# MatchaChoco010/toy-cpu-pathtracing

Measured on AMD Instinct MI355X. Metric: Msamples/sec (whole node), scene3 MIS/Sobol 1920x1080, higher is better.
Workload: dtype f32; 1 GPU; scene3 1920x1080 mis+sobol, 1024-spp job, 1024 sample indices per step (BASELINE configs[1]); parallelism=single-gpu

## Files before the change

toy-cpu-pathtracing_amd/csrc/api.cpp:

```cpp
#include <hip/hip_runtime.h>

#include <algorithm>
#include <cmath>
#include <cstdio>
#include <cstring>
#include <string>
#include <vector>

#include "../../include/mi355pt.h"
#include "api_internal.hpp"

using namespace pt;

static thread_local std::string g_err;
bool pt::g_debug_unlocked = false;
int pt::fail(int code, const std::string& msg) { g_err = msg; return code; }

static const uint32_t CIE_CMF_BITS[470 * 4] = {
#include "cie_cmf.inc"
};
void pt::cie_cmf4(float out[470 * 4]) { std::memcpy(out, CIE_CMF_BITS, sizeof(CIE_CMF_BITS)); }

namespace {

// ... 64 lines not shown
}

static void free_parts(std::vector<MultiPart>& parts) {
    for (size_t i = 0; i < parts.size(); ++i) {
        MultiPart& m = parts[i];
        (void)hipSetDevice(m.device);
        if (m.stream) (void)hipStreamDestroy(m.stream);
        if (m.done) (void)hipEventDestroy(m.done);
        (void)hipFree(m.d_film); (void)hipFree(m.d_pack); (void)hipFree(m.d_stage); (void)hipFree(m.d_out);
        if (i > 0) delete m.scene;
    }
    parts.clear();
}
mi355pt_scene::~mi355pt_scene() {
    int cur = 0;
    const bool have = !parts.empty() && hipGetDevice(&cur) == hipSuccess;
    free_parts(parts);
    if (have) (void)hipSetDevice(cur);
    delete ctx;
}

static int launch_range(const mi355pt_scene* s, const mi355pt_camera* cam, const mi355pt_params* p, uint32_t s_begin, uint32_t s_end, float* d_accum,
                        hipStream_t stream, mi355pt_stats* stats, const PathOut& pout, int aov_kind, uint32_t illuminant_lut, const uint32_t* d_list,
                        uint32_t n_list) {
    const bool aov = aov_kind >= 0;
    if (!d_list && shard_tile_count(cam->width, cam->height, p->shard_index, p->shard_count) == 0) return MI355PT_OK;
    int rc;
    LaunchCtx* lc; int slot;
    if ((rc = get_launch_ctx(s, p->seed, &lc, &slot))) return rc;
    if (lc->device != s->impl.device) return fail(MI355PT_E_DEVICE, "launch context and scene live on different devices");
    const bool want_stats = stats && p->collect_stats;
    int& waves = aov ? lc->aov_waves[aov_kind] : lc->waves[want_stats ? 1 : 0][p->sampler & 1u][p->strategy < 3u ? p->strategy : 0u];
    if (!waves) waves = aov ? query_resident_waves_aov((uint32_t)aov_kind, s->impl.features)
                            : query_resident_waves(select_kernel(false, want_stats, s->impl.features, p->sampler, p->strategy));
    const DevCamera dc = make_camera(cam);
    LaunchPlan plan = d_list ? plan_launch_tiles(cam, p, s_begin, s_end, waves, n_list) : plan_launch(cam, p, s_begin, s_end, waves, aov);
    DevParams& dp = plan.params;
    if (d_list) set_tile_list(dp, d_list);
    unsigned* d_counter = lc->d_counters + slot;
    DevStats* d_stats = lc->d_stats + slot;
    HIP_TRY(hipMemsetAsync(d_counter, 0, sizeof(unsigned), stream));
    dp.stats_mode = p->collect_stats;
    if (want_stats || (aov && stats)) HIP_TRY(hipMemsetAsync(d_stats, 0, sizeof(DevStats), stream));
    hipEvent_t e0 = nullptr, e1 = nullptr;
    if (stats) { HIP_TRY(hipEventCreate(&e0)); HIP_TRY(hipEventCreate(&e1)); HIP_TRY(hipEventRecord(e0, stream)); }
    if ((rc = grow_device_buffer(&lc->d_partial, &lc->partial_bytes, plan.partial_floats * sizeof(float), stream))) return rc;
    const KernelKey key = select_kernel(d_list != nullptr, want_stats, s->impl.features, p->sampler, p->strategy);
    if ((rc = grow_device_buffer(&lc->d_defer, &lc->defer_bytes, aov ? (size_t)0 : query_defer_bytes_per_wave(key) * (size_t)plan.grid, stream))) return rc;
    if (aov) HIP_TRY(launch_aov((uint32_t)aov_kind, s->impl.dev, dc, dp, illuminant_lut, lc->d_hash, d_accum, d_counter, stats ? d_stats : nullptr,
                                s->impl.features, plan.grid, stream));
    else {
        DevScene dev = s->impl.dev;
        dev.cam_lists = use_camera_lists(key, dp.block_log2, camera_lists_enabled()) ? 1u : 0u;
        HIP_TRY(launch_pt(key, dev, dc, dp, plan.n_tiles,
                          lc->d_hash, d_accum, lc->d_partial, d_counter, d_list ? nullptr : d_stats, plan.grid, stream, pout, lc->d_defer));
    }
    if (stats) {
        HIP_TRY(hipEventRecord(e1, stream));
        HIP_TRY(hipEventSynchronize(e1));
        float ms = 0.0f;
        HIP_TRY(hipEventElapsedTime(&ms, e0, e1));
        std::memset(stats, 0, sizeof(*stats));
        stats->kernel_ms = ms; stats->launches = 1;
        if (want_stats || aov) {
            DevStats h;
            HIP_TRY(hipMemcpy(&h, d_stats, sizeof(h), hipMemcpyDeviceToHost));
            copy_stats(h, stats);
        }
        (void)hipEventDestroy(e0); (void)hipEventDestroy(e1);
    }
    return MI355PT_OK;
}

static int launch_ranges(const mi355pt_scene* s, const mi355pt_camera* cam, const mi355pt_params* p, uint32_t s_begin, uint32_t s_end, float* d_accum,
                         hipStream_t stream, mi355pt_stats* stats, const uint32_t* d_list, uint32_t n_list,
                         const PathOut& pout = PathOut{nullptr, nullptr, nullptr, 0u, 0u}, int aov_kind = -1, uint32_t illuminant_lut = 0) {
    return for_each_launch_range(p->sampler, stats != nullptr, s_begin, s_end, [&](uint32_t b, uint32_t e) {
        return launch_range(s, cam, p, b, e, d_accum, stream, stats, pout, aov_kind, illuminant_lut, d_list, n_list);
    });
}

int pt::render_accum_range(const mi355pt_scene* s, const mi355pt_camera* cam, const mi355pt_params* p, uint32_t s_begin, uint32_t s_end,
                           float* d_accum, void* hip_stream, mi355pt_stats* stats, const PathOut& pout, int aov_kind, uint32_t illuminant_lut) {
    const bool aov = aov_kind >= 0;
    int rc = check_args(s, cam, p, aov);
    if (rc) return rc;
    if (!d_accum || s_end > p->spp || s_begin >= s_end) return fail(MI355PT_E_INVALID, "bad sample range or null accumulator");
    if (aov) {
        if (aov_kind > MI355PT_AOV_SHADING_NORMAL) return fail(MI355PT_E_INVALID, "unknown AOV kind");
        if (p->collect_stats) return fail(MI355PT_E_INVALID, "the AOV renderers have no instrumented kernel: collect_stats must be 0");
        if (aov_kind == MI355PT_AOV_ALBEDO && illuminant_lut >= s->impl.luts.size())
            return fail(MI355PT_E_INVALID, "illuminant_lut is not a LUT470 id of this scene (presets::cie_illum_d6500())");
    }
    return launch_ranges(s, cam, p, s_begin, s_end, d_accum, (hipStream_t)hip_stream, stats, nullptr, 0u, pout, aov_kind, illuminant_lut);
}

static int check_tiles_args(const mi355pt_scene* s, const mi355pt_camera* cam, const mi355pt_params* p) {
    int rc = check_args(s, cam, p);
    if (rc) return rc;
    if (p->shard_count > 1u) return fail(MI355PT_E_INVALID, "tile lists name tiles of the whole frame: shard_count must be 0 or 1");
    if (p->collect_stats) return fail(MI355PT_E_INVALID, "there is no instrumented tile-list kernel: collect_stats must be 0");
    if (adaptive_tile_count(cam->width, cam->height) == 0u) return fail(MI355PT_E_INVALID, "the frame has 2^31 tiles or more");
    return MI355PT_OK;
}

extern "C" {
// ... 693 lines not shown
```

toy-cpu-pathtracing_amd/csrc/launch_plan.hpp:

```cpp
#pragma once
#include <algorithm>
#include <cmath>
#include <cstddef>
#include <cstdint>
#include <cstdlib>

#include "../../include/mi355pt.h"
#include "layout.hpp"

namespace pt {

struct V3 { float x, y, z; };
inline V3 cross3(V3 a, V3 b) { return {a.y * b.z - b.y * a.z, a.z * b.x - b.z * a.x, a.x * b.y - b.x * a.y}; }
inline V3 norm3(V3 a) { float r = 1.0f / std::sqrt((a.x * a.x) + (a.y * a.y) + (a.z * a.z)); return {a.x * r, a.y * r, a.z * r}; }

inline uint32_t log2_int(uint32_t v) { return v == 0 ? 0 : 31 - (uint32_t)__builtin_clz(v); }
inline uint32_t round_up_pow2(uint32_t v) { return v <= 1 ? 1 : 1u << (32 - __builtin_clz(v - 1)); }

inline uint32_t shard_tile_count(uint32_t width, uint32_t height, uint32_t shard_index, uint32_t shard_count) {
    const uint32_t total = ((width + 7) / 8) * ((height + 7) / 8);
    const uint32_t cnt = shard_count ? shard_count : 1u, idx = shard_count ? shard_index : 0u;
    return total > idx ? (total - idx + cnt - 1) / cnt : 0u;
}

// ... 100 lines not shown
    while (!aov && n_items * chunks < (uint32_t)waves * 8 && chunks * 2 <= n_samples &&
           (n_samples / (chunks * 2)) >= (n_items * chunks >= (uint32_t)waves ? 16u : 8u)) chunks *= 2;
#ifdef MI355PT_TUNING
    if (const char* e = getenv("MI355PT_CHUNKS")) { uint32_t c = (uint32_t)atoi(e); if (c >= 1 && c <= n_samples) chunks = c; }
#endif
    dp.chunks = chunks; dp.chunk_size = (n_samples + chunks - 1) / chunks;
    dp.n_work = n_items * chunks;
    dp.sample_prefix_digits = 0;
    if (dp.sampler == MI355PT_SAMPLER_SOBOL && block_log2 == 0 && (dp.log2_spp & 1u) == 0u && n_samples % chunks == 0) {
        const uint32_t cs = dp.chunk_size;
        uint32_t m = 0;
        while ((1u << (2u * (m + 1u))) <= cs) ++m;
        if ((1u << (2u * m)) == cs && s_begin % cs == 0 && m >= 3 && m <= dp.log2_spp / 2u &&
            2u * dp.n_base4_digits <= 2u * m + 27u) dp.sample_prefix_digits = dp.log2_spp / 2u - m;
    }
    const int grid = (int)std::min<uint32_t>(dp.n_work, (uint32_t)waves);
    return LaunchPlan{dp, n_tiles, grid, dp.chunks > 1 ? (size_t)n_tiles * dp.chunks * 64u * 3u : (size_t)0};
}
inline LaunchPlan plan_launch(const mi355pt_camera* cam, const mi355pt_params* p, uint32_t s_begin, uint32_t s_end, int waves, bool aov) {
    return plan_launch_over(cam, p, s_begin, s_end, waves, aov, shard_tile_count(cam->width, cam->height, p->shard_index, p->shard_count));
}
inline LaunchPlan plan_launch_tiles(const mi355pt_camera* cam, const mi355pt_params* p, uint32_t s_begin, uint32_t s_end, int waves, uint32_t n_list) {
    return plan_launch_over(cam, p, s_begin, s_end, waves, false, n_list);
}

enum : uint32_t { MODE_GENERIC = 0, MODE_MIS_SOBOL = 1, MODE_NEE_SOBOL = 2, MODE_PT = 3, MODE_COUNT = 4 };
#define PT_FOR_EACH_SET(P, C)                                                                                                          \
    P(0u) P(FEAT_TEX) P(FEAT_DIEL) P(FEAT_METAL) P(FEAT_DIEL | FEAT_ROUGH) P(FEAT_DELTA | FEAT_MLIGHT) P(FEAT_STD & ~FEAT_CC)           \
    C(FEAT_CC) C(FEAT_CC | FEAT_TEX) C(FEAT_STD) C(FEAT_ALL)
#define PT_NO_SET(F)
#define PT_FOR_EACH_PLAIN_SET(X) PT_FOR_EACH_SET(X, PT_NO_SET)
#define PT_FOR_EACH_CC_SET(X) PT_FOR_EACH_SET(PT_NO_SET, X)
#define PT_SET_ENTRY(F) (F),
inline constexpr uint32_t FEATURE_SETS[] = {PT_FOR_EACH_SET(PT_SET_ENTRY, PT_SET_ENTRY)};
inline constexpr uint32_t PLAIN_SETS[] = {PT_FOR_EACH_PLAIN_SET(PT_SET_ENTRY)};
inline constexpr uint32_t CC_SETS[] = {PT_FOR_EACH_CC_SET(PT_SET_ENTRY)};
#undef PT_SET_ENTRY
inline uint32_t pick_features(uint32_t feat) {
    for (uint32_t s : FEATURE_SETS) if ((feat & ~s) == 0u) return s;
    return FEAT_ALL;
}
struct KernelKey { bool tiles, stats; uint32_t mode, set; };
inline KernelKey select_kernel(bool tiles, bool stats, uint32_t feat, uint32_t sampler, uint32_t strategy) {
    if (stats) return KernelKey{tiles, true, MODE_GENERIC, (feat & (FEAT_CC | FEAT_EMTEX)) == 0u ? FEAT_STD & ~FEAT_CC : FEAT_ALL};
    const uint32_t mode = sampler == MI355PT_SAMPLER_SOBOL && strategy == MI355PT_STRATEGY_MIS ? MODE_MIS_SOBOL
                        : sampler == MI355PT_SAMPLER_SOBOL && strategy == MI355PT_STRATEGY_NEE ? MODE_NEE_SOBOL
                        : strategy == MI355PT_STRATEGY_PT ? MODE_PT : MODE_GENERIC;
    return KernelKey{tiles, false, mode, pick_features(feat)};
}

inline bool use_camera_lists(const KernelKey& key, uint32_t block_log2, bool enabled) { return enabled && !key.stats && block_log2 <= 3u; }
inline bool camera_lists_enabled() { const char* e = getenv("MI355PT_NO_CAMERA_LISTS"); return !(e && e[0] != '\0' && !(e[0] == '0' && e[1] == '\0')); }

}
```

toy-cpu-pathtracing_amd/csrc/layout.hpp:

```cpp
#pragma once
#include <stddef.h>
#include <stdint.h>

#if defined(__HIPCC__)
#define PT_HD __host__ __device__
#else
#define PT_HD
#endif

namespace pt {

#ifndef PT_STACK_DEPTH
#define PT_STACK_DEPTH 24
#endif
constexpr int STACK_DEPTH = PT_STACK_DEPTH;
constexpr int MAX_LEAF_TRIS = 4;
constexpr int MAX_BUILD_DEPTH = 22;
constexpr int HASH_TABLE_DIMS = 136;

struct alignas(16) DevNode {
    float bx[4];
    float by[4];
    float bz[4];
    int32_t child[2];
// ... 107 lines not shown
    uint32_t material;
    float area_sum;
    uint32_t kind;
    float intensity;
    float angle_inner, angle_outer;
    float pos[3];
    float pad0;
    float axis[3];
    float pad1;
};
static_assert(sizeof(DevLight) == 64, "light record");

struct DevEnv {
    const float* texels;
    const float* marginal;
    const float* conditional;
    uint32_t w, h;
    float total_weight, intensity;
    float l2r[9], r2l[9];
    uint32_t illuminant_lut;
    uint32_t light_index;
    uint32_t pad[2];
};

struct DevScene {
    const DevNode* nodes;
    const DevNode4* nodes4;
    const DevNode4Q* nodes4q;
    float grid_org[3], grid_cell[3];
    const DevTri* tris;
    const DevTriShade* shade;
    const DevTriLocal* tris_local;
    const DevTri* tris_render;
    float tri_shift[3]; uint32_t tris_are_local;
    float shared_mw[3]; uint32_t pad_mw;
    const DevInstance* instances;
    const DevMaterial* materials;
    const DevLight* lights;
    const DevLightTri* light_tris;
    const float* light_uvs;
    const float* luts;
    const float* cmf;
    const float* rgb2spec;
    const float* z_nodes;
    const uint32_t* texels;
    const DevTexture* textures;
    const float* cc_albedo;
    uint32_t n_nodes, n_tris, n_lights, n_materials;
    int32_t root;
    int32_t root4;
    uint32_t n_nodes4;
    uint32_t cam_lists;
    const DevEnv* envs;
    uint32_t n_envs, pad_env;
};

struct DevCamera {
    float s[3], u[3], f[3];
    float tan_half_fov, aspect;
    uint32_t width, height;
};

struct DevParams {
    uint32_t spp, seed, max_depth, strategy, sampler;
    float exposure;
    uint32_t log2_spp, n_base4_digits;
    uint32_t sample_begin, sample_end;
    uint32_t shard_index, shard_count;
    uint32_t tiles_x, tiles_y;
    uint32_t n_work;
    uint32_t chunks, chunk_size;
    uint32_t block_log2;
    uint32_t sample_prefix_digits;
    uint32_t stats_mode;
    uint32_t albedo_lut;
    float rr_gate;
    float xyz_to_rgb[9];
};
static_assert(offsetof(DevParams, shard_index) == 40 && offsetof(DevParams, shard_count) == 44, "the shard pair carries the tile-list pointer");
PT_HD inline void set_tile_list(DevParams& p, const uint32_t* list) {
    p.shard_index = (uint32_t)((uint64_t)(uintptr_t)list & 0xffffffffu); p.shard_count = (uint32_t)((uint64_t)(uintptr_t)list >> 32);
}
PT_HD inline const uint32_t* tile_list(const DevParams& p) { return (const uint32_t*)(uintptr_t)(((uint64_t)p.shard_count << 32) | p.shard_index); }

enum : uint32_t { FEAT_TEX = 1, FEAT_DIEL = 2, FEAT_CC = 4, FEAT_MLIGHT = 8, FEAT_ROUGH = 16, FEAT_METAL = 32, FEAT_DELTA = 64, FEAT_ENV = 128, FEAT_EMTEX = 256,
                  FEAT_STD = 255, FEAT_ALL = 511 };

struct DevStats {
    unsigned long long samples, closest_rays, shadow_rays, nodes_closest, tris_closest, nodes_shadow, tris_shadow;
    unsigned long long closest_hits, bounces, spectrum_evals, textured_lookups;
    unsigned long long phase_cycles[10];
    unsigned long long wave_steps[8];
    unsigned long long busy_hist[2][8];
    unsigned long long divergence[12];
};

}
```

toy-cpu-pathtracing_amd/csrc/pt_kernel_body.inc:

```
    __shared__ uint32_t s_stack[STACK_DEPTH * 64];
#ifndef PT_FILM_PIX
#define PT_FILM_PIX 64
#endif
    __shared__ float s_film[PT_FILM_PIX * 3];
    __shared__ uint32_t s_hi[SOBOL_HI_DIMS];
    __shared__ uint32_t s_p6[SOBOL_HI_DIMS];
    __shared__ unsigned s_work;
    constexpr bool PARK = (FEAT & FEAT_CC) != 0u && kernel_min_waves<FEAT>() <= 3;
    __shared__ float s_park[PARK ? 8 * 64 : 1];
    __shared__ uint8_t s_perm[96];
    __shared__ uint32_t s_ring[ANY_RING];
    __shared__ uint32_t s_occl[2];
    __shared__ uint32_t s_pair[64];
    const AnyLds any_lds{s_ring, s_occl, s_pair};
    __shared__ unsigned long long s_best[64];
    const ClosestLds closest_lds{s_ring, s_best, s_pair};
    __shared__ uint32_t s_infl[2];
    const PairLds pair_lds{s_ring, s_best, s_occl, s_pair, s_infl};
    constexpr bool CAMLIST = !STATS && tail_queue<FEAT, MODE>();
    __shared__ uint32_t s_cand[CAMLIST ? CAM_LIST_CAP : 1u];
    DevParams prm = prm_in;
    if constexpr (MODE == MODE_MIS_SOBOL) { prm.strategy = 2u; prm.sampler = 1u; }
    if constexpr (MODE == MODE_NEE_SOBOL) { prm.strategy = 1u; prm.sampler = 1u; }
    if constexpr (MODE == MODE_PT) prm.strategy = 0u;
    const uint32_t lane = threadIdx.x;
    auto park = [&](Path& Q, bool mine = true) {
        if constexpr (PARK) {
            if (mine) {
#pragma unroll
                for (int i = 0; i < 4; ++i) s_park[i * 64 + lane] = Q.pf[i];
                s_park[4 * 64 + lane] = Q.p_pdf; s_park[5 * 64 + lane] = Q.prev_pos.x; s_park[6 * 64 + lane] = Q.prev_pos.y; s_park[7 * 64 + lane] = Q.prev_pos.z;
            }
#pragma unroll
            for (int i = 0; i < 4; ++i) Q.pf[i] = 0.0f;
            Q.p_pdf = 0.0f; Q.prev_pos = mk3(0.0f, 0.0f, 0.0f);
        }
    };
    auto unpark = [&](Path& Q) {
        if constexpr (PARK) {
#pragma unroll
            for (int i = 0; i < 4; ++i) Q.pf[i] = s_park[i * 64 + lane];
            Q.p_pdf = s_park[4 * 64 + lane]; Q.prev_pos = mk3(s_park[5 * 64 + lane], s_park[6 * 64 + lane], s_park[7 * 64 + lane]);
        }
    };
    uint32_t* stack = s_stack + lane;
    for (uint32_t k = lane; k < 96u; k += 64u) s_perm[k] = (uint8_t)((perm_packed(k >> 2) >> (2u * (k & 3u))) & 3u);
    if constexpr ((FEAT & (FEAT_TEX | FEAT_EMTEX | FEAT_ENV)) != 0u) s_znodes[lane] = sc.z_nodes[lane];
    __syncthreads();
    SamplerCtx sctx{prm.sampler, prm.seed, prm.log2_spp, prm.n_base4_digits, cam.width, dim_hash_tab, nullptr, 0u, 0u, nullptr, s_perm};
    StatCounters st{};
    unsigned long long tp[10] = {0, 0, 0, 0, 0, 0, 0, 0, 0, 0};
    unsigned long long dvc[8] = {0, 0, 0, 0, 0, 0, 0, 0};
    unsigned long long t_loop0 = 0;
// ... 3 lines not shown
        if (lane == 0) s_work = atomicAdd(work_counter, 1u);
        __syncthreads();
        const uint32_t work = s_work;
        __syncthreads();
        if (work >= prm.n_work) break;
        const LaneJob job = PT_LANE_JOB(work, lane, cam, prm);
        const LaneJob job0 = PT_LANE_JOB(work, 0u, cam, prm);
        const uint32_t blk_log2 = prm.block_log2, blk_mask = (1u << blk_log2) - 1u;
        const uint32_t s_prefix = prm.sample_prefix_digits;
        const uint32_t hi_first_w = sobol_hi_first(prm.log2_spp, blk_log2) - s_prefix, hi_shift_w = 2u * hi_first_w - (prm.log2_spp & 1u);
        if (prm.sampler == 1u && hi_first_w < prm.n_base4_digits && hi_first_w >= 3u &&
            2u * prm.n_base4_digits - (prm.log2_spp & 1u) <= hi_shift_w + 27u) {
            sctx.hi_first = sobol_hi_first(prm.log2_spp, blk_log2) - s_prefix;
            sctx.hi_shift = 2u * sctx.hi_first - (prm.log2_spp & 1u);
            const uint32_t tile_m = (encode_morton2_u32(job0.px, job0.py) << prm.log2_spp) | (s_prefix ? job0.s_cur : 0u);
            for (uint32_t dmn = lane; dmn < (uint32_t)SOBOL_HI_DIMS; dmn += 64) {
                uint32_t e = (uint32_t)(sobol_tile_hi_digits(tile_m, dmn, prm.log2_spp, prm.n_base4_digits, sctx.hi_first) >> sctx.hi_shift);
                const uint64_t prefix = (uint64_t)tile_m >> sctx.hi_shift;
                e |= sobol_perm_index(prefix, dmn) << 27;
                uint32_t e6 = 0;
                for (uint32_t v7 = 0; v7 < 4u; ++v7) e6 |= sobol_perm_index((prefix << 2) | v7, dmn) << (5u * v7);
                s_hi[dmn] = e; s_p6[dmn] = e6;
            }
            sctx.hi_lds = s_hi; sctx.p6_lds = s_p6;
        }
        uint32_t cam_n = CAM_LIST_NONE;
        if constexpr (CAMLIST) {
            if (sc.cam_lists != 0u) {
                const uint32_t x0 = PT_CAM_UNIFORM(job0.px), y0 = PT_CAM_UNIFORM(job0.py);
                const CamWalk cw = cam_walk(sc.nodes4, sc.root4, sc.tris, sc.tri_shift, cam_pyramid(cam, x0, y0, x0 + blk_mask, y0 + blk_mask), s_cand, CAM_LIST_CAP, s_ring);
                cam_n = PT_CAM_UNIFORM(cw.overflow ? CAM_LIST_NONE : cw.count);
            }
        }
        if (lane < PT_FILM_PIX) { s_film[3 * lane] = 0.0f; s_film[3 * lane + 1] = 0.0f; s_film[3 * lane + 2] = 0.0f; }
        __syncthreads();
        const uint32_t n_s = job0.s_end > job0.s_cur ? job0.s_end - job0.s_cur : 0u;
        const uint32_t pool_size = n_s << (2u * blk_log2);
        uint32_t pool_next = 0u;
        uint32_t my_pix = lane;
        Path P{};
        park(P);
        bool active = false;
        constexpr bool MERGED = merged_traversal<FEAT, MODE>();
        ShadowReq sh{};
        bool dying = false, susp = false;
        CarryState carry{0ull};
        constexpr bool TAILQ = !STATS && tail_queue<FEAT, MODE>();
        constexpr uint32_t DEFER = TAILQ ? 0u : defer_classes<FEAT, MODE>();
        float4* const q_base = (DEFER != 0u || TAILQ) ? defer_buf + (size_t)blockIdx.x * (queue_bytes_per_wave(STATS, FEAT, MODE) / 16u) : nullptr;
        uint32_t q_head = 0u, q_tail = 0u;
        uint32_t q_count = 0u, q2_count = 0u;
        constexpr uint32_t TQ_CLASSES = (TAILQ && (FEAT & FEAT_CC) != 0u) ? ((1u << MT_CLEARCOAT) | (1u << (MT_CLEARCOAT | 8u))) : 0u;
        constexpr uint32_t QR = (TQ_CLASSES != 0u) ? QUEUE_RING : PT_TAILQ_RING1;
        while (true) {
            unsigned long long ts0 = 0, ts1 = 0, ts2 = 0, ts3 = 0, ts4 = 0, tsa = 0, tsb = 0;
            uint32_t bsdf_classes = 0u;
            if (STATS) ts0 = __builtin_amdgcn_s_memtime();
            bool popped = false;
            uint32_t pop_e = 0u;
            const unsigned long long m_needy = __ballot(!active);
            if (m_needy != 0ull && pool_next < pool_size) {
                const uint32_t idx = pool_next + rank_below(m_needy);
                if (!active && idx < pool_size) {
                    const uint32_t pix = idx & ((1u << (2u * blk_log2)) - 1u);
                    const uint32_t px = job0.px + (pix & blk_mask), py = job0.py + (pix >> blk_log2);
                    const uint32_t smp_i = job0.s_cur + (idx >> (2u * blk_log2));
                    const bool valid = px < cam.width && py < cam.height;
                    if (valid) { active = true; my_pix = pix; regen_path<STATS>(P, sctx, cam, px, py, smp_i, st); }
                }
                pool_next = min(pool_next + (uint32_t)__popcll(m_needy), pool_size);
            }
            if (!__any(active)) {
                if (pool_next >= pool_size && q_tail == q_head && (q_count | q2_count) == 0u) break;
                if (!((DEFER != 0u || TAILQ) && pool_next >= pool_size)) continue;
            }
            if (STATS) { ts1 = __builtin_amdgcn_s_memtime(); if (lane == 0) st.w[4]++; if (active) st.w[5]++; }
            Hit hit{};
            bool got = false;
            const bool canonical = STATS && prm.stats_mode == 1u;
            if (canonical) { if (active) got = trace_closest<STATS>(sc, P.ro, P.rd, 3.402823466e+38f, stack, hit, st); }
            else if constexpr (MERGED) {
                bool occluded = false;
                if (STATS && sh.on) st.w[6]++;
                bool cam_ray = false;
                if constexpr (CAMLIST) cam_ray = cam_n != CAM_LIST_NONE && active && !dying && P.from_camera && P.depth == 0u;
                if (!CAMLIST || __ballot((active && !dying && !popped && !cam_ray) || sh.on) != 0ull) {
                    PT_PRIO_TRAV_ENTER;
                    trace_pair_coop<STATS>(sc, P.ro, P.rd, active && !dying && !popped && !cam_ray, sh.o, sh.d, sh.t, sh.on, stack, lane, pair_lds, hit, got, occluded, st, &carry, susp, &susp);
                    PT_PRIO_TRAV_EXIT;
                }
                if constexpr (CAMLIST) {
                    if (__ballot(cam_ray) != 0ull) {
                        const RaySetup rs = setup_ray(P.rd);
                        const f3 o2 = tri_origin(sc, P.ro);
                        unsigned long long key = (0x7f7fffffull << 32) | 0xffffffffull;
                        for (uint32_t i = 0u; i < cam_n; ++i) {
                            const uint32_t tri = PT_CAM_UNIFORM(s_cand[i]);
                            const TriVerts tv = load_tri(sc.tris, tri);
                            float t, b0, b1, b2;
                            if (intersect_triangle<false>(o2, P.rd, rs.kx, rs.ky, rs.kz, rs.sx, rs.sy, rs.sz, 3.402823466e+38f, tv, t, b0, b1, b2)) {
                                const unsigned long long k = ((unsigned long long)__float_as_uint(t) << 32) | (unsigned long long)tri;
                                key = k < key ? k : key;
                            }
                        }
                        if (cam_ray) {
                            got = (uint32_t)key != 0xffffffffu;
                            if (got) winner_hit(sc, P.ro, P.rd, rs, (uint32_t)key, hit);
                        }
                    }
                }
                if (sh.on && !occluded) {
#pragma unroll
                    for (int i = 0; i < 4; ++i) P.L[i] = P.L[i] + sh.c[i];
                }
                sh = ShadowReq{};
            }
            else { PT_PRIO_TRAV_ENTER; got = trace_closest_coop<STATS>(sc, P.ro, P.rd, active, stack, lane, closest_lds, hit, st); PT_PRIO_TRAV_EXIT; }
            if (STATS) {
                const uint32_t mclass = (active && got) ? sc.materials[__float_as_uint(((const float4*)(sc.shade + hit.tri))[4].z)].type : 8u;
                uint32_t classes = 0u, largest = 0u, lanes = 0u;
                for (uint32_t c = 0u; c < 8u; ++c) {
                    const uint32_t n = (uint32_t)__popcll(__ballot(mclass == c));
                    classes += n ? 1u : 0u; largest = max(largest, n); lanes += n;
                }
                if (lane == 0 && lanes) { st.dv[0]++; st.dv[1] += classes; st.dv[2] += lanes; st.dv[3] += largest; }
                bsdf_classes = classes - (__ballot(mclass == MT_EMISSIVE) != 0ull ? 1u : 0u);
                ts2 = __builtin_amdgcn_s_memtime();
            }
            auto tq_store = [&](uint32_t e, const Path& Q, const Hit& h, uint32_t pix) {
                float4* r = q_base + (size_t)(e >> 8) * (TQ_F4 * QUEUE_RING) + (e & (QR - 1u));
                const uint32_t fl = (Q.wl.term ? 1u : 0u) | ((Q.depth & 1023u) << 1) | ((pix & 63u) << 11) | (Q.smp.dimension << 17);
                r[0u * QR] = make_float4(__uint_as_float(Q.smp.morton), __uint_as_float(fl), Q.wl.lam0, __uint_as_float(h.tri));
                r[1u * QR] = make_float4(Q.T[0], Q.T[1], Q.T[2], Q.T[3]);
                r[2u * QR] = make_float4(Q.L[0], Q.L[1], Q.L[2], Q.L[3]);
                r[3u * QR] = make_float4(Q.rd.x, Q.rd.y, Q.rd.z, h.b0);
                r[4u * QR] = make_float4(h.b1, h.b2, __uint_as_float(Q.smp.rkey_lo), __uint_as_float(Q.smp.rkey_hi));
            };
            auto tq_load = [&](uint32_t e, Path& Q, Hit& h, uint32_t& pix) {
                const float4* r = q_base + (size_t)(e >> 8) * (TQ_F4 * QUEUE_RING) + (e & (QR - 1u));
                const float4 a = r[0u * QR], b = r[1u * QR], c = r[2u * QR], d = r[3u * QR], e4 = r[4u * QR];
                const uint32_t fl = __float_as_uint(a.y);
                Q.smp.morton = __float_as_uint(a.x); Q.smp.dimension = fl >> 17; Q.smp.rkey_lo = __float_as_uint(e4.z); Q.smp.rkey_hi = __float_as_uint(e4.w);
                Q.wl.lam0 = a.z; Q.wl.term = (fl & 1u) != 0u; Q.depth = (fl >> 1) & 1023u; pix = (fl >> 11) & 63u;
                Q.from_camera = false; Q.prev_spec = false;
                Q.T[0] = b.x; Q.T[1] = b.y; Q.T[2] = b.z; Q.T[3] = b.w; Q.L[0] = c.x; Q.L[1] = c.y; Q.L[2] = c.z; Q.L[3] = c.w;
                Q.rd = mk3(d.x, d.y, d.z); Q.ro = mk3(0.0f, 0.0f, 0.0f);
                h.b0 = d.w; h.b1 = e4.x; h.b2 = e4.y; h.tri = __float_as_uint(a.w); h.mclass = 0u; h.t = 0.0f;
#pragma unroll
                for (int i = 0; i < 4; ++i) Q.pf[i] = 0.0f;
                Q.p_pdf = 0.0f; Q.prev_pos = mk3(0.0f, 0.0f, 0.0f);
            };
            auto dq_store = [&](uint32_t e, const Path& Q, const Hit& h, uint32_t pix) {
                float4* r = q_base + (size_t)e * DEFER_F4;
                const uint32_t fl = (Q.wl.term ? 1u : 0u) | (Q.from_camera ? 2u : 0u) | (Q.prev_spec ? 4u : 0u) | ((Q.depth & 1023u) << 3) | (pix << 16);
                r[0] = make_float4(__uint_as_float(Q.smp.morton), __uint_as_float(Q.smp.dimension), __uint_as_float(Q.smp.rkey_lo), __uint_as_float(Q.smp.rkey_hi));
                r[1] = make_float4(Q.wl.lam0, __uint_as_float(fl), Q.T[0], Q.T[1]);
                r[2] = make_float4(Q.T[2], Q.T[3], Q.L[0], Q.L[1]);
                r[3] = make_float4(Q.L[2], Q.L[3], Q.rd.x, Q.rd.y);
                r[4] = make_float4(Q.rd.z, Q.pf[0], Q.pf[1], Q.pf[2]);
                r[5] = make_float4(Q.pf[3], Q.p_pdf, Q.prev_pos.x, Q.prev_pos.y);
                r[6] = make_float4(Q.prev_pos.z, h.t, h.b0, h.b1);
                r[7] = make_float4(h.b2, __uint_as_float(h.tri), __uint_as_float(h.mclass), 0.0f);
            };
            auto dq_load = [&](uint32_t e, Path& Q, Hit& h, uint32_t& pix) {
                const float4* r = q_base + (size_t)e * DEFER_F4;
                const float4 a = r[0], b = r[1], c = r[2], d = r[3], e4 = r[4], f = r[5], g = r[6], h4 = r[7];
                const uint32_t fl = __float_as_uint(b.y);
                Q.smp.morton = __float_as_uint(a.x); Q.smp.dimension = __float_as_uint(a.y); Q.smp.rkey_lo = __float_as_uint(a.z); Q.smp.rkey_hi = __float_as_uint(a.w);
                Q.wl.lam0 = b.x; Q.wl.term = (fl & 1u) != 0u; Q.from_camera = (fl & 2u) != 0u; Q.prev_spec = (fl & 4u) != 0u; Q.depth = (fl >> 3) & 1023u; pix = fl >> 16;
                Q.T[0] = b.z; Q.T[1] = b.w; Q.T[2] = c.x; Q.T[3] = c.y; Q.L[0] = c.z; Q.L[1] = c.w; Q.L[2] = d.x; Q.L[3] = d.y;
                Q.rd = mk3(d.z, d.w, e4.x); Q.ro = mk3(0.0f, 0.0f, 0.0f);
                Q.pf[0] = e4.y; Q.pf[1] = e4.z; Q.pf[2] = e4.w; Q.pf[3] = f.x; Q.p_pdf = f.y; Q.prev_pos = mk3(f.z, f.w, g.x);
                h.t = g.y; h.b0 = g.z; h.b1 = g.w; h.b2 = h4.x; h.tri = __float_as_uint(h4.y); h.mclass = __float_as_uint(h4.z);
            };
            auto finish_path = [&]() {
                if (pout.L != nullptr) {
                    const uint32_t px = job0.px + (my_pix & blk_mask), py = job0.py + (my_pix >> blk_log2);
                    const uint32_t tile_k = (work / prm.chunks) >> (6u - 2u * blk_log2);
                    const uint32_t smp_i = P.smp.morton & ((1u << prm.log2_spp) - 1u);
                    sample_log(P, pout, ((size_t)tile_k * 64u + ((py & 7u) * 8u + (px & 7u))) * pout.n_s + (smp_i - pout.s_base));
                }
                float r, g, b;
                film_rgb(P, sc, prm, r, g, b);
                atomicAdd(&s_film[3 * my_pix], r); atomicAdd(&s_film[3 * my_pix + 1], g); atomicAdd(&s_film[3 * my_pix + 2], b);
            };
            if constexpr (TAILQ) {
                bool end_path = dying;
                const bool front = active && !dying && !susp;
                unpark(P);
                {
                    ShadeCtx C0;
                    C0.cont = false;
                    if (front) end_path = shade_vertex_head<STATS, FEAT, 1>(P, sc, prm, sctx, got, hit, sh, st, tsa, C0);
                }
                dying = false;
                const bool go_on = front && !end_path;
                const bool cls2 = TQ_CLASSES != 0u && ((TQ_CLASSES >> (hit.mclass & 31u)) & 1u) != 0u;
                const unsigned long long m_on1 = __ballot(go_on && !cls2), m_on2 = TQ_CLASSES != 0u ? __ballot(go_on && cls2) : 0ull;
                if ((m_on1 | m_on2) != 0ull) {
                    if (go_on) {
                        const uint32_t e = cls2 ? QUEUE_RING + tq_push_slot(q2_count, rank_below(m_on2)) : tq_push_slot(q_count, rank_below(m_on1));
                        tq_store(e, P, hit, my_pix);
                        active = false;
                    }
                    q_count += (uint32_t)__popcll(m_on1); q2_count += (uint32_t)__popcll(m_on2);
                    __builtin_amdgcn_fence(__ATOMIC_RELEASE, "workgroup");
                }
                if (active && end_path) { finish_path(); active = false; }
                park(P, false);
                if (STATS) ts3 = ts4 = __builtin_amdgcn_s_memtime();
                const bool draining = pool_next >= pool_size;
                if (tq_pass_due(q_count, q2_count, draining, TQ_CLASSES != 0u, (uint32_t)PT_TAILQ_MIN)) {
                    const unsigned long long m_free = __ballot(!active);
                    const uint32_t n_free = (uint32_t)__popcll(m_free), r = rank_below(m_free);
                    const TqTake tk = tq_pass_take(q_count, q2_count, n_free, draining, TQ_CLASSES != 0u, (uint32_t)PT_TAILQ_MIN);
                    const uint32_t n2 = tk.n2, n1 = tk.n1;
                    const bool take2 = !active && r < n2, take1 = !active && !take2 && r - n2 < n1;
                    const bool take = take1 || take2;
                    const uint32_t e = take2 ? QUEUE_RING + tq_pop_slot(q2_count, n2, r) : tq_pop_slot(q_count, n1, r - n2);
                    q2_count -= n2; q_count -= n1;
                    bool ep = false;
                    if constexpr ((FEAT & FEAT_CC) != 0u) {
                        ShadeCtx C;
                        shade_ctx_idle_cc(C);
                        if (take) {
                            __builtin_amdgcn_fence(__ATOMIC_ACQUIRE, "workgroup");
                            tq_load(e, P, hit, my_pix);
                            active = true;
                            shade_vertex_head<STATS, FEAT, 2>(P, sc, prm, sctx, true, hit, sh, st, tsa, C);
                        }
                        const bool want_mc = take && C.cont && C.need_cc;
                        const float fc_mc = coat_directional_albedo_coop(want_mc, C.cc_alpha_c, C.cc_r0c, C.wo_nm, C.mc_key, lane);
                        if (want_mc) C.cc_fc = fc_mc;
                        if (take && C.cont) ep = shade_vertex_tail<STATS, FEAT>(P, sc, prm, sctx, sh, st, tsb, C);
                    } else if (take) {
                        __builtin_amdgcn_fence(__ATOMIC_ACQUIRE, "workgroup");
                        tq_load(e, P, hit, my_pix);
                        active = true;
                        ShadeCtx C;
                        C.cont = false; C.need_cc = false; C.cc_fc = 0.0f;
                        shade_vertex_head<STATS, FEAT, 2>(P, sc, prm, sctx, true, hit, sh, st, tsa, C);
                        if (C.cont) ep = shade_vertex_tail<STATS, FEAT>(P, sc, prm, sctx, sh, st, tsb, C);
                    }
                    park(P, take);
                    if (sh.on && sh.c[0] == 0.0f && sh.c[1] == 0.0f && sh.c[2] == 0.0f && sh.c[3] == 0.0f) sh.on = false;
                    if (!active) sh.on = false;
                    if (take) { dying = sh.on && ep; if (dying) ep = false; }
                    if (take && ep) { finish_path(); active = false; }
                }
            } else
            for (int pass = 0;; ++pass) {
            const bool mine = pass == 0 || popped;
            bool end_path = pass == 0 && MERGED && dying;
            if (pass == 0) {
                if constexpr (!MERGED) sh = ShadowReq{};
                unpark(P);
            }
            if constexpr (DEFER != 0u) {
                if (popped) {
                    __builtin_amdgcn_fence(__ATOMIC_ACQUIRE, "workgroup");
                    dq_load(pop_e, P, hit, my_pix);
                    got = true;
                }
                const bool defer_now = pass == 0 && !(STATS && prm.stats_mode == 1u) && active && !dying && !susp && !popped && got && ((DEFER >> (hit.mclass & 31u)) & 1u) != 0u;
                const unsigned long long m_def = __ballot(defer_now);
                if (m_def != 0ull) {
                    if (defer_now) {
                        dq_store((q_tail + rank_below(m_def)) & (DEFER_RING - 1u), P, hit, my_pix);
                        active = false;
                    }
                    q_tail += (uint32_t)__popcll(m_def);
                    __builtin_amdgcn_fence(__ATOMIC_RELEASE, "workgroup");
                }
            }
            const bool shade_now = mine && active && !(MERGED && (dying || susp));
            if constexpr ((FEAT & FEAT_CC) != 0u) {
                ShadeCtx C;
                shade_ctx_idle_cc(C);
                if (shade_now) end_path = shade_vertex_head<STATS, FEAT>(P, sc, prm, sctx, got, hit, sh, st, tsa, C);
                const bool want_mc = shade_now && C.cont && C.need_cc;
                const float fc_mc = coat_directional_albedo_coop(want_mc, C.cc_alpha_c, C.cc_r0c, C.wo_nm, C.mc_key, lane);
                if (want_mc) C.cc_fc = fc_mc;
                if (shade_now && C.cont) end_path = shade_vertex_tail<STATS, FEAT>(P, sc, prm, sctx, sh, st, tsb, C);
            } else {
                if (shade_now) end_path = shade_vertex<STATS, FEAT>(P, sc, prm, sctx, got, hit, sh, st, tsa, tsb);
            }
            park(P, mine);
            if (STATS) {
                ts3 = __builtin_amdgcn_s_memtime();
                unsigned long long ma = __ballot(tsa != 0ull), mb = __ballot(tsb != 0ull);
// ... 76 lines not shown
```

toy-cpu-pathtracing_amd/csrc/scene_lower.cpp:

```cpp
#include "scene_lower.hpp"

#include <algorithm>
#include <cfloat>
#include <cmath>
#include <cstdio>
#include <cstring>

namespace pt {

namespace {

constexpr float PI_F = 3.14159265358979323846f;

struct V3 { float x, y, z; };
inline V3 operator-(V3 a, V3 b) { return {a.x - b.x, a.y - b.y, a.z - b.z}; }
inline V3 cross(V3 a, V3 b) { return {a.y * b.z - b.y * a.z, a.z * b.x - b.z * a.x, a.x * b.y - b.x * a.y}; }
inline float dot(V3 a, V3 b) { return (a.x * b.x) + (a.y * b.y) + (a.z * b.z); }
inline float length(V3 a) { return std::sqrt(dot(a, a)); }
inline V3 normalize(V3 a) { float r = 1.0f / length(a); return {a.x * r, a.y * r, a.z * r}; }
inline V3 vertex(const HostMesh& mesh, uint32_t v) { return V3{mesh.pos[3 * v], mesh.pos[3 * v + 1], mesh.pos[3 * v + 2]}; }
inline bool degenerate(V3 a, V3 b, V3 c) { const V3 cr = cross(b - a, c - a); return dot(cr, cr) == 0.0f; }

template <typename Rec>
inline void set_vertices(Rec& r, V3 a, V3 b, V3 c) {
// ... 547 lines not shown
    dev.n_envs = (uint32_t)ls->envs.size();
    dev.n_nodes = (uint32_t)ls->nodes.size(); dev.n_tris = (uint32_t)ls->tris_render.size();
    dev.n_lights = (uint32_t)ls->lights.size(); dev.n_materials = (uint32_t)ls->materials.size();
    dev.root = bvh.root;
    rep->n_degenerate = g.n_degenerate;
    rep->bvh_depth = bvh.max_depth;
    return MI355PT_OK;
}

int lower_tree4(LoweredScene* ls, LowerReport* rep, std::string* err) {
    std::vector<DevNode4> nodes4;
    if (!collapse_bvh4(ls->nodes, ls->dev.root, ls->tris_render.size(), &nodes4, &ls->dev.root4, &rep->stack_need, err, &rep->collapse_method)) return MI355PT_E_INVALID;
    ls->dev.n_nodes4 = (uint32_t)nodes4.size();
#if PT_NODE_FMA
    pad_nodes4(&nodes4);
#endif
#if PT_NODE_Q16
    if (!quantise_nodes4(nodes4, ls->dev.grid_org, ls->dev.grid_cell, &ls->nodes4, err)) return MI355PT_E_INVALID;
#else
    ls->nodes4 = std::move(nodes4);
#endif
    return MI355PT_OK;
}

std::string lowering_info(const LoweredScene& ls, const LowerReport& rep, bool gpu_builder, const double* ms) {
    char t_bvh[64] = "", t_collapse[32] = "", tail[160];
    if (ms) { std::snprintf(t_bvh, sizeof(t_bvh), " bvh_ms=%.2f bvh_device_ms=%.2f", ms[0], ms[1]); std::snprintf(t_collapse, sizeof(t_collapse), " collapse_ms=%.2f", ms[2]); }
    std::snprintf(tail, sizeof(tail), " stack_need=%d/%d degenerate=%zu tri_space=%s features=%u", rep.stack_need, STACK_DEPTH, rep.n_degenerate,
                  ls.dev.tris_are_local ? "local" : "render", ls.features);
    return "nodes4=" + std::to_string(ls.dev.n_nodes4) + " nodes=" + std::to_string(ls.nodes.size()) + " tris=" + std::to_string(ls.tris_render.size()) +
           " depth=" + std::to_string(rep.bvh_depth) + " builder=" + (gpu_builder ? "gpu" : "host") + t_bvh + " collapse=" + rep.collapse_method + t_collapse + tail;
}

void lowering_digests(const LoweredScene& ls, const LowerReport& rep, std::vector<std::string>* names, std::vector<uint64_t>* digests) {
    names->clear(); digests->clear();
    auto add = [&](const std::string& name, const void* p, size_t bytes) { names->push_back(name); digests->push_back(fnv1a64(p, bytes)); };
#define PT_DIGEST(v) add(#v, ls.v.data(), ls.v.size() * sizeof(ls.v[0]))
    PT_DIGEST(nodes); PT_DIGEST(nodes4); PT_DIGEST(tris_render); PT_DIGEST(shade); PT_DIGEST(instances); PT_DIGEST(tris_local); PT_DIGEST(cc_albedo);
    PT_DIGEST(materials); PT_DIGEST(lights); PT_DIGEST(light_tris); PT_DIGEST(light_uvs); PT_DIGEST(luts); PT_DIGEST(cmf); PT_DIGEST(rgb2spec);
    PT_DIGEST(z_nodes); PT_DIGEST(texels); PT_DIGEST(textures);
#undef PT_DIGEST
    for (size_t k = 0; k < ls.env_tables.size(); ++k) {
        const LoweredScene::EnvTables& t = ls.env_tables[k];
        const std::string e = "env" + std::to_string(k);
        add(e + ".texels", t.texels.data(), t.texels.size() * 4); add(e + ".marginal", t.marginal.data(), t.marginal.size() * 4);
        add(e + ".conditional", t.conditional.data(), t.conditional.size() * 4);
    }
    add("envs", ls.envs.data(), ls.envs.size() * sizeof(DevEnv));
    std::string b;
    auto put = [&](const void* p, size_t n) { b.append((const char*)p, n); };
    const DevScene& dev = ls.dev;
    put(dev.grid_org, 12); put(dev.grid_cell, 12); put(dev.tri_shift, 12); put(&dev.tris_are_local, 4); put(dev.shared_mw, 12); put(&dev.pad_mw, 4);
    put(&dev.n_nodes, 4); put(&dev.n_tris, 4); put(&dev.n_lights, 4); put(&dev.n_materials, 4); put(&dev.root, 4); put(&dev.root4, 4);
    put(&dev.n_nodes4, 4); put(&dev.cam_lists, 4); put(&dev.n_envs, 4); put(&dev.pad_env, 4);
    const uint32_t feat = ls.features; const uint64_t ndeg = rep.n_degenerate, nn4 = dev.n_nodes4; const int32_t depth = rep.bvh_depth, need = rep.stack_need;
    put(&feat, 4); put(&ndeg, 8); put(&depth, 4); put(&nn4, 8); put(&need, 4); put(rep.collapse_method, std::strlen(rep.collapse_method));
    add("scalars", b.data(), b.size());
}

}
```

toy-cpu-pathtracing_amd/csrc/tail_queue_plan.hpp:

```cpp
#pragma once
#include <cstdint>

namespace pt {

constexpr uint32_t tq_push_slot(uint32_t count, uint32_t rank) { return count + rank; }
constexpr uint32_t tq_pop_slot(uint32_t count, uint32_t n, uint32_t rank) { return count - n + rank; }

struct TqTake { uint32_t n1, n2; };

constexpr bool tq_pass_due(uint32_t c1, uint32_t c2, bool draining, bool two_queues, uint32_t pass_min) {
    return (two_queues && c2 >= pass_min) || c1 >= pass_min || (draining && (c1 | c2) != 0u);
}
constexpr TqTake tq_pass_take(uint32_t c1, uint32_t c2, uint32_t n_free, bool draining, bool two_queues, uint32_t pass_min) {
    const bool full2 = two_queues && c2 >= pass_min, full1 = c1 >= pass_min;
    const uint32_t n2 = (full2 || (draining && !full1)) ? (n_free < c2 ? n_free : c2) : 0u;
    const uint32_t n1 = (!full2 || draining) ? (n_free - n2 < c1 ? n_free - n2 : c1) : 0u;
    return TqTake{n1, n2};
}

}
```

Baseline: 2701 Msamples/s.

## Stage tail-queue pushes in LDS when a pass is due immediately

When the lanes pushed in this iteration would trigger a tail-queue pass straight away, their path records go into the LDS traversal-stack buffer instead of the global-memory ring. The following pop then reads those records back from LDS and the rest from global memory, which skips a global write and read round trip for records that are consumed at once. The LDS stack is reused as scratch, so its ordering against traversal has to stay correct. The staging is on by default for non-stats kernels with a single queue and can be turned off with an environment variable.

```diff
diff --git a/toy-cpu-pathtracing_amd/csrc/api.cpp b/toy-cpu-pathtracing_amd/csrc/api.cpp
--- a/toy-cpu-pathtracing_amd/csrc/api.cpp
+++ b/toy-cpu-pathtracing_amd/csrc/api.cpp
@@ -140,6 +140,7 @@
     else {
         DevScene dev = s->impl.dev;
         dev.cam_lists = use_camera_lists(key, dp.block_log2, camera_lists_enabled()) ? 1u : 0u;
+        dev.queue_stage = use_queue_staging(key, queue_staging_enabled()) ? 1u : 0u;
         HIP_TRY(launch_pt(key, dev, dc, dp, plan.n_tiles,
                           lc->d_hash, d_accum, lc->d_partial, d_counter, d_list ? nullptr : d_stats, plan.grid, stream, pout, lc->d_defer));
     }
diff --git a/toy-cpu-pathtracing_amd/csrc/launch_plan.hpp b/toy-cpu-pathtracing_amd/csrc/launch_plan.hpp
--- a/toy-cpu-pathtracing_amd/csrc/launch_plan.hpp
+++ b/toy-cpu-pathtracing_amd/csrc/launch_plan.hpp
@@ -176,4 +176,7 @@
 inline bool use_camera_lists(const KernelKey& key, uint32_t block_log2, bool enabled) { return enabled && !key.stats && block_log2 <= 3u; }
 inline bool camera_lists_enabled() { const char* e = getenv("MI355PT_NO_CAMERA_LISTS"); return !(e && e[0] != '\0' && !(e[0] == '0' && e[1] == '\0')); }
 
+inline bool use_queue_staging(const KernelKey& key, bool enabled) { return enabled && !key.stats; }
+inline bool queue_staging_enabled() { const char* e = getenv("MI355PT_NO_QUEUE_STAGING"); return !(e && e[0] != '\0' && !(e[0] == '0' && e[1] == '\0')); }
+
 }
diff --git a/toy-cpu-pathtracing_amd/csrc/layout.hpp b/toy-cpu-pathtracing_amd/csrc/layout.hpp
--- a/toy-cpu-pathtracing_amd/csrc/layout.hpp
+++ b/toy-cpu-pathtracing_amd/csrc/layout.hpp
@@ -183,7 +183,8 @@
     uint32_t n_nodes4;
     uint32_t cam_lists;
     const DevEnv* envs;
-    uint32_t n_envs, pad_env;
+    uint32_t n_envs;
+    uint32_t queue_stage;
 };
 
 struct DevCamera {
diff --git a/toy-cpu-pathtracing_amd/csrc/pt_kernel_body.inc b/toy-cpu-pathtracing_amd/csrc/pt_kernel_body.inc
--- a/toy-cpu-pathtracing_amd/csrc/pt_kernel_body.inc
+++ b/toy-cpu-pathtracing_amd/csrc/pt_kernel_body.inc
@@ -1,4 +1,4 @@
-    __shared__ uint32_t s_stack[STACK_DEPTH * 64];
+    __shared__ __attribute__((aligned(16))) uint32_t s_stack[STACK_DEPTH * 64];
 #ifndef PT_FILM_PIX
 #define PT_FILM_PIX 64
 #endif
@@ -108,6 +108,9 @@
         uint32_t q_count = 0u, q2_count = 0u;
         constexpr uint32_t TQ_CLASSES = (TAILQ && (FEAT & FEAT_CC) != 0u) ? ((1u << MT_CLEARCOAT) | (1u << (MT_CLEARCOAT | 8u))) : 0u;
         constexpr uint32_t QR = (TQ_CLASSES != 0u) ? QUEUE_RING : PT_TAILQ_RING1;
+        constexpr bool STAGE = TAILQ && TQ_CLASSES == 0u;
+        static_assert(STACK_DEPTH * 64 >= (int)(TQ_STAGE_SLOTS * TQ_F4 * 4u) && TQ_STAGE_SLOTS == 64u, "a pass's worth of staged tail-queue records fits the traversal stack's LDS");
+        float4* const s_stage = (float4*)s_stack;
         while (true) {
             unsigned long long ts0 = 0, ts1 = 0, ts2 = 0, ts3 = 0, ts4 = 0, tsa = 0, tsb = 0;
             uint32_t bsdf_classes = 0u;
@@ -183,18 +186,21 @@
                 bsdf_classes = classes - (__ballot(mclass == MT_EMISSIVE) != 0ull ? 1u : 0u);
                 ts2 = __builtin_amdgcn_s_memtime();
             }
+            auto tq_put = [&](float4* r, uint32_t stride, const Path& Q, const Hit& h, uint32_t pix) {
+                const uint32_t fl = (Q.wl.term ? 1u : 0u) | ((Q.depth & 1023u) << 1) | ((pix & 63u) << 11) | (Q.smp.dimension << 17);
+                r[0u * stride] = make_float4(__uint_as_float(Q.smp.morton), __uint_as_float(fl), Q.wl.lam0, __uint_as_float(h.tri));
+                r[1u * stride] = make_float4(Q.T[0], Q.T[1], Q.T[2], Q.T[3]);
+                r[2u * stride] = make_float4(Q.L[0], Q.L[1], Q.L[2], Q.L[3]);
+                r[3u * stride] = make_float4(Q.rd.x, Q.rd.y, Q.rd.z, h.b0);
+                r[4u * stride] = make_float4(h.b1, h.b2, __uint_as_float(Q.smp.rkey_lo), __uint_as_float(Q.smp.rkey_hi));
+            };
             auto tq_store = [&](uint32_t e, const Path& Q, const Hit& h, uint32_t pix) {
-                float4* r = q_base + (size_t)(e >> 8) * (TQ_F4 * QUEUE_RING) + (e & (QR - 1u));
-                const uint32_t fl = (Q.wl.term ? 1u : 0u) | ((Q.depth & 1023u) << 1) | ((pix & 63u) << 11) | (Q.smp.dimension << 17);
-                r[0u * QR] = make_float4(__uint_as_float(Q.smp.morton), __uint_as_float(fl), Q.wl.lam0, __uint_as_float(h.tri));
-                r[1u * QR] = make_float4(Q.T[0], Q.T[1], Q.T[2], Q.T[3]);
-                r[2u * QR] = make_float4(Q.L[0], Q.L[1], Q.L[2], Q.L[3]);
-                r[3u * QR] = make_float4(Q.rd.x, Q.rd.y, Q.rd.z, h.b0);
-                r[4u * QR] = make_float4(h.b1, h.b2, __uint_as_float(Q.smp.rkey_lo), __uint_as_float(Q.smp.rkey_hi));
-            };
-            auto tq_load = [&](uint32_t e, Path& Q, Hit& h, uint32_t& pix) {
-                const float4* r = q_base + (size_t)(e >> 8) * (TQ_F4 * QUEUE_RING) + (e & (QR - 1u));
-                const float4 a = r[0u * QR], b = r[1u * QR], c = r[2u * QR], d = r[3u * QR], e4 = r[4u * QR];
+                tq_put(q_base + (size_t)(e >> 8) * (TQ_F4 * QUEUE_RING) + (e & (QR - 1u)), QR, Q, h, pix);
+            };
+            struct TqRec { float4 a, b, c, d, e4; };
+            auto tq_get = [&](const float4* r, uint32_t stride) { return TqRec{r[0u * stride], r[1u * stride], r[2u * stride], r[3u * stride], r[4u * stride]}; };
+            auto tq_unpack = [&](const TqRec& rec, Path& Q, Hit& h, uint32_t& pix) {
+                const float4 a = rec.a, b = rec.b, c = rec.c, d = rec.d, e4 = rec.e4;
                 const uint32_t fl = __float_as_uint(a.y);
                 Q.smp.morton = __float_as_uint(a.x); Q.smp.dimension = fl >> 17; Q.smp.rkey_lo = __float_as_uint(e4.z); Q.smp.rkey_hi = __float_as_uint(e4.w);
                 Q.wl.lam0 = a.z; Q.wl.term = (fl & 1u) != 0u; Q.depth = (fl >> 1) & 1023u; pix = (fl >> 11) & 63u;
@@ -205,6 +211,9 @@
 #pragma unroll
                 for (int i = 0; i < 4; ++i) Q.pf[i] = 0.0f;
                 Q.p_pdf = 0.0f; Q.prev_pos = mk3(0.0f, 0.0f, 0.0f);
+            };
+            auto tq_load = [&](uint32_t e, Path& Q, Hit& h, uint32_t& pix) {
+                tq_unpack(tq_get(q_base + (size_t)(e >> 8) * (TQ_F4 * QUEUE_RING) + (e & (QR - 1u)), QR), Q, h, pix);
             };
             auto dq_store = [&](uint32_t e, const Path& Q, const Hit& h, uint32_t pix) {
                 float4* r = q_base + (size_t)e * DEFER_F4;
@@ -253,10 +262,19 @@
                 const bool go_on = front && !end_path;
                 const bool cls2 = TQ_CLASSES != 0u && ((TQ_CLASSES >> (hit.mclass & 31u)) & 1u) != 0u;
                 const unsigned long long m_on1 = __ballot(go_on && !cls2), m_on2 = TQ_CLASSES != 0u ? __ballot(go_on && cls2) : 0ull;
+                uint32_t n_on1 = 0u;
+                bool stage = false;
+                if constexpr (STAGE) {
+                    n_on1 = (uint32_t)__popcll(m_on1);
+                    stage = sc.queue_stage != 0u && tq_stage_pushes(q_count, n_on1, pool_next >= pool_size, (uint32_t)PT_TAILQ_MIN);
+                }
                 if ((m_on1 | m_on2) != 0ull) {
                     if (go_on) {
-                        const uint32_t e = cls2 ? QUEUE_RING + tq_push_slot(q2_count, rank_below(m_on2)) : tq_push_slot(q_count, rank_below(m_on1));
-                        tq_store(e, P, hit, my_pix);
+                        if (STAGE && stage) tq_put(s_stage + tq_stage_push_index(rank_below(m_on1)), TQ_STAGE_SLOTS, P, hit, my_pix);
+                        else {
+                            const uint32_t e = cls2 ? QUEUE_RING + tq_push_slot(q2_count, rank_below(m_on2)) : tq_push_slot(q_count, rank_below(m_on1));
+                            tq_store(e, P, hit, my_pix);
+                        }
                         active = false;
                     }
                     q_count += (uint32_t)__popcll(m_on1); q2_count += (uint32_t)__popcll(m_on2);
@@ -274,6 +292,8 @@
                     const bool take2 = !active && r < n2, take1 = !active && !take2 && r - n2 < n1;
                     const bool take = take1 || take2;
                     const uint32_t e = take2 ? QUEUE_RING + tq_pop_slot(q2_count, n2, r) : tq_pop_slot(q_count, n1, r - n2);
+                    TqStagePop sp{0u, false, 0u};
+                    if constexpr (STAGE) sp = tq_stage_pop(stage ? q_count - n_on1 : q_count, stage ? n_on1 : 0u, n1, r - n2);
                     q2_count -= n2; q_count -= n1;
                     bool ep = false;
                     if constexpr ((FEAT & FEAT_CC) != 0u) {
@@ -291,7 +311,11 @@
                         if (take && C.cont) ep = shade_vertex_tail<STATS, FEAT>(P, sc, prm, sctx, sh, st, tsb, C);
                     } else if (take) {
                         __builtin_amdgcn_fence(__ATOMIC_ACQUIRE, "workgroup");
-                        tq_load(e, P, hit, my_pix);
+                        static_assert(STAGE, "the kernels without the clearcoat code have one queue");
+                        TqRec rec;
+                        if (!sp.staged) rec = tq_get(q_base + sp.slot, QR);
+                        else rec = tq_get(s_stage + sp.index, TQ_STAGE_SLOTS);
+                        tq_unpack(rec, P, hit, my_pix);
                         active = true;
                         ShadeCtx C;
                         C.cont = false; C.need_cc = false; C.cc_fc = 0.0f;
diff --git a/toy-cpu-pathtracing_amd/csrc/scene_lower.cpp b/toy-cpu-pathtracing_amd/csrc/scene_lower.cpp
--- a/toy-cpu-pathtracing_amd/csrc/scene_lower.cpp
+++ b/toy-cpu-pathtracing_amd/csrc/scene_lower.cpp
@@ -623,7 +623,7 @@
     const DevScene& dev = ls.dev;
     put(dev.grid_org, 12); put(dev.grid_cell, 12); put(dev.tri_shift, 12); put(&dev.tris_are_local, 4); put(dev.shared_mw, 12); put(&dev.pad_mw, 4);
     put(&dev.n_nodes, 4); put(&dev.n_tris, 4); put(&dev.n_lights, 4); put(&dev.n_materials, 4); put(&dev.root, 4); put(&dev.root4, 4);
-    put(&dev.n_nodes4, 4); put(&dev.cam_lists, 4); put(&dev.n_envs, 4); put(&dev.pad_env, 4);
+    put(&dev.n_nodes4, 4); put(&dev.cam_lists, 4); put(&dev.n_envs, 4); put(&dev.queue_stage, 4);
     const uint32_t feat = ls.features; const uint64_t ndeg = rep.n_degenerate, nn4 = dev.n_nodes4; const int32_t depth = rep.bvh_depth, need = rep.stack_need;
     put(&feat, 4); put(&ndeg, 8); put(&depth, 4); put(&nn4, 8); put(&need, 4); put(rep.collapse_method, std::strlen(rep.collapse_method));
     add("scalars", b.data(), b.size());
diff --git a/toy-cpu-pathtracing_amd/csrc/tail_queue_plan.hpp b/toy-cpu-pathtracing_amd/csrc/tail_queue_plan.hpp
--- a/toy-cpu-pathtracing_amd/csrc/tail_queue_plan.hpp
+++ b/toy-cpu-pathtracing_amd/csrc/tail_queue_plan.hpp
@@ -18,4 +18,17 @@
     return TqTake{n1, n2};
 }
 
+constexpr uint32_t TQ_STAGE_SLOTS = 64u;
+
+constexpr bool tq_stage_pushes(uint32_t count, uint32_t n_push, bool draining, uint32_t pass_min) {
+    return n_push != 0u && tq_pass_due(count + n_push, 0u, draining, false, pass_min);
 }
+constexpr uint32_t tq_stage_push_index(uint32_t rank) { return rank; }
+
+struct TqStagePop { uint32_t slot; bool staged; uint32_t index; };
+constexpr TqStagePop tq_stage_pop(uint32_t count, uint32_t n_push, uint32_t n_take, uint32_t rank) {
+    const uint32_t slot = tq_pop_slot(count + n_push, n_take, rank);
+    return TqStagePop{slot, slot >= count, slot >= count ? slot - count : 0u};
+}
+
+}
```

Result: faster. 2755 Msamples/s (median of 6 runs) (+2.0%).
